# waiwera/waiwera

Hardware: AMD Instinct MI355X
Metric: Newton steps/sec, 10M-cell eos_we (BCSR SpMV GB/s in roofline) (higher is better)
Workload: dtype f64

## Files before the change

### include/waiwera_hip_bench.h

```cpp
#ifndef WAIWERA_HIP_BENCH_H
#define WAIWERA_HIP_BENCH_H
#include "waiwera_hip.h"
#ifdef __cplusplus
extern "C" {
#endif

int wai_comm_stats(wai_ctx *ctx, long long *allreduces, long long *exchanges);
int wai_gather_stats(wai_ctx *ctx, long long *gathers);
int wai_launch_stats(wai_ctx *ctx, long long *kernels, long long *copies);
int wai_tracer_stats(wai_ctx *ctx, long long *assembly_sweeps);

int wai_bench_mute_comm(wai_ctx *ctx, int on);
int wai_test_drop_partials(wai_ctx *ctx, int n);
int wai_test_drop_stream_wait(wai_ctx *ctx, int which);
int wai_test_device_memory(long long *allocations, long long *bytes);
int wai_test_pc_operator(wai_ctx *ctx, int spmv, const double *x, const double *x2, double alpha, int dot_mode,
                         const double *aux, int split, int fin_phase, const double *scal_in, double *z, double *scal_out);
int wai_pc_axpy_capable(wai_ctx *ctx);
int wai_test_partial_count(wai_ctx *ctx);
int wai_test_desc_templates(wai_ctx *ctx, int *bricks, int *rows);
enum { WAI_KV_DOT = 0, WAI_KV_DOTS, WAI_KV_WAXPY, WAI_KV_BCGS_P, WAI_KV_BCGS_S, WAI_KV_BCGS_XR, WAI_KV_BCGS_XRP,
       WAI_KV_BCGS_XRP_DERIVE, WAI_KV_SCALARS, WAI_KV_MDOT, WAI_KV_MAXPY_NORM, WAI_KV_SCALE_TO, WAI_KV_UPDATE_X };
int wai_test_krylov_vec(wai_ctx *ctx, int op, int variant, int n, int k, long long ld, long long len, double alpha,
                        double *vecs, double *basis, const double *coef, double *scal, double *post);
int wai_halo_size(wai_ctx *ctx, int dof, long long *bytes_sent, int *n_neighbours);

int wai_timer_start(wai_ctx *ctx);
int wai_timer_stop(wai_ctx *ctx, float *ms);
int wai_bench_kernel(wai_ctx *ctx, int which, int reps, float *ms_per_launch);
int wai_bcgs_composed(wai_ctx *ctx);
int wai_profile_enable(wai_ctx *ctx, int on);
int wai_profile_get(wai_ctx *ctx, int kclass, double *ms, long long *launches);
int wai_profile_reset(wai_ctx *ctx);

#ifdef __cplusplus
}
#endif
#endif
```

### waiwera_amd/csrc/context.hpp

```cpp
#pragma once
#include <hip/hip_runtime.h>
#include <string>
#include <type_traits>
#include <vector>
#include "../../include/waiwera_hip.h"
#include "devbuf.hpp"
#include "ilu_schedule.hpp"
#include "mesh_pattern.hpp"
#include "physics.hip.h"

namespace wai {

__host__ __device__ __forceinline__ size_t ell_ld(size_t n) {
  size_t ld = (n + 511) & ~(size_t)511;
  if ((ld & 262143) == 0) ld += 512;
  return ld;
}
__host__ __device__ __forceinline__ size_t ell_rows(int bs, size_t n) {
  if (bs >= 3) return ell_ld(n);
  return n;
}
__host__ __device__ __forceinline__ size_t ell_ix1(int bs, size_t n, int r, int k, size_t i) {
  if (bs >= 3) return ((i >> 6) * (size_t)(bs * bs) + (size_t)(r * bs + k)) * 64 + (i & 63);
  return ((size_t)r * n + i) * bs + k;
// ... 119 lines not shown
  std::vector<int> h_rowptr, h_colidx;
};

struct LinSys;
struct IluSchedule : ScheduleFacts {
  DevBuf<int> sub_ptr;
  DevBuf<int> sub_nlev;
  DevBuf<int> sub_split;
  DevBuf<int> row_info;
  DevBuf<unsigned long long> row_infow;
  DevBuf<double> fval;
  DevBuf<double> dinv;
  DevBuf<int> row_uoff;
  DevBuf<int> row_tslot;
  DevBuf<int> sub_int;
  DevBuf<int> sub_bnd;
  DevBuf<int> sub_order;
  DevBuf<int> row_uoffw;
  DevBuf<unsigned short> col16;
  DevBuf<int> sub_seg;
  DevBuf<int> t_info, t_uoff;
  DevBuf<unsigned short> t_col16;
  DevBuf<int> sub_desc;
  DevBuf<int> ord_f;
  DevBuf<int> ord_b;
  const LinSys* owner = nullptr;
};
inline int pc_threads(const IluSchedule& s) { return ((s.max_rows + 63) / 64) * 64; }

template <class F>
int with_bs(int bs, F&& f) {
  switch (bs) {
    case 1: f(std::integral_constant<int, 1>{}); return 0;
    case 2: f(std::integral_constant<int, 2>{}); return 0;
    case 3: f(std::integral_constant<int, 3>{}); return 0;
    case 4: f(std::integral_constant<int, 4>{}); return 0;
    default: return -1;
  }
}
template <class F>
void with_flag(bool flag, F&& f) {
  if (flag) f(std::true_type{});
  else f(std::false_type{});
}
template <class F>
int with_eos(int kind, F&& f) {
// ... 176 lines not shown
  wai::Network net;
  std::vector<int> src_gidx;
  int src_nglobal = 0;
  wai::Pattern pat;
  wai::LinSys flow, aux, coupled;
  wai::KrylovVecs kv, kv_coupled;
  wai::IluSchedule ilu;
  wai::LuBlocks lu;
  wai::Krylov ks;
  wai::Tracers tr;
  wai::Gather gat;
  wai::DevBuf<double> tr_bc, tr_inj, tr_rhsb;
  wai::DevBuf<double> flu, flu_last_iter, flu_last_step, flu_pert;
  wai::DevBuf<double> hstep;
  wai::DevBuf<double> w_y, w_yold, w_delta, w_f, w_lhs, w_a, w_b, w_c;
  wai::DevBuf<int> d_flags;
  wai::PinnedBuf<int> h_flags;
  wai::DevBuf<double> d_red;
  wai::PinnedBuf<double> h_red;
  wai::DevBuf<double> stage[4];
  size_t stage_len = 0;
  struct EnvSw {
    bool fin_separate = false; bool no_col16 = false; bool scalar_kernels = false; bool iluk_level_path = false;
    bool asm_unfused = false; bool no_desc_share = false;
  } env;
  int test_drop_wait = 0;
  int n_nbr = 0;
  std::vector<int> nbr_rank, send_ptr, recv_ptr;
  wai::DevBuf<int> d_send_idx; wai::DevBuf<double> d_sendbuf, d_recvbuf;
  int send_total = 0, max_dof_buf = 0;
  double fnorm0 = 0.0;
  int method = 0;
  double ratio = 0.0;
  wai::DevBuf<double> w_lhs2;
  int scheme = 0, taken = 0;
  double dt_last = 0.0;
  wai::DevBuf<double> w_hist;
  wai::DevBuf<double> w_hist_prev;
  double dt_last_prev = 0.0;
  bool can_reject = false;
  bool prof_on = false;
  bool last_iter_partial = false;
  double prof_ms[wai::KC_COUNT] = {0};
  long long prof_n[wai::KC_COUNT] = {0};
  std::string err;
  bool bc_set = false;
  int dbg = 0;
// ... 80 lines not shown
```

### waiwera_amd/csrc/ilu_schedule.hpp

```cpp
#pragma once
#include <algorithm>
#include <numeric>
#include <string>
#include <unordered_map>
#include <vector>

namespace wai {

struct ScheduleFacts {
  int nsub = 0, max_rows = 0, max_lev = 0;
  std::vector<int> sub;
  bool wide = false;
  bool diag_only = false;
  bool scaled = true;
  bool park = true;
  int max_nl = 0;
  int n_int = 0, n_bnd = 0;
  int max_ublocks = 0;
  int max_ublocks_w = 0;
  bool fast3 = false;
  int max_nlu = 0;
  bool rows_kernel = false;
  bool wave_kernel = false;
  int n_templates = 0, template_rows = 0;
  bool big = false;
  bool sublu = false;
  int nlev_f = 0, nlev_b = 0;
  std::vector<int> lev_f_ptr, lev_b_ptr;
};

struct HostSchedule : ScheduleFacts {
  std::vector<int> nlev;
  std::vector<int> info;
  std::vector<unsigned long long> infow;
  std::vector<int> uoff;
  std::vector<int> uoffw;
  std::vector<int> tslot;
  std::vector<int> split;
  std::vector<int> order;
  std::vector<int> sub_int, sub_bnd;
  std::vector<int> ord_f, ord_b;
  std::vector<unsigned short> c16;
  std::vector<int> seg;
  std::vector<int> t_info, t_uoff;
  std::vector<unsigned short> t_c16;
  std::vector<int> desc;
};

struct ScheduleOpts {
  bool ghosts = false;
  bool allow_wide = true, sublu = false, fill = false;
  int mesh_W = 0;
  bool box_faces = false;
  int max_seg = 8;
  bool ilu_general = false;
  int pc_rows = -1;
  bool pc_wave = true;
};

struct ScheduleCsr {
  const std::vector<int>& rowptr;
  const std::vector<int>& colidx;
  const int* row(int i) const { return colidx.data() + rowptr[i]; }
  int count(int i) const { return rowptr[i + 1] - rowptr[i]; }
};
struct ScheduleRows {
  std::vector<int> diag, lfirst, ulast, levf, levb;
  int max_nu = 0, nlf_all = 0, nlb_all = 0;
  bool offdiag_fill = false;
// ... 51 lines not shown
      const int k = row[q];
      const int* rk = A.row(k);
      const int* e = std::lower_bound(rk + r.diag[k] + 1, rk + r.ulast[k], i);
      const int r2 = (e < rk + r.ulast[k] && *e == i) ? (int)(e - rk) : 15;
      pack |= (r2 & 15) << (4 * p);
    }
    out.tslot[i] = pack;
    out.max_nl = std::max(out.max_nl, r.diag[i] - r.lfirst[i]);
  }
}

inline void sub_upper_offsets(int lo, int hi, ScheduleRows& r, HostSchedule& out) {
  int ucount = 0, ucountw = 0;
  for (int i = lo; i < hi; i++) {
    const int nL = r.diag[i] - r.lfirst[i], nU = r.ulast[i] - r.diag[i] - 1;
    if (nL > 3 || nU > 3 || r.lfirst[i] > 3 || r.diag[i] > 3) out.fast3 = false;
    out.max_nlu = std::max(out.max_nlu, std::max(nL, nU));
    out.uoff[i] = ucount;
    ucount += std::min(nU, 3);
    out.uoffw[i] = ucountw;
    ucountw += nU;
    r.max_nu = std::max(r.max_nu, nU);
  }
  out.max_ublocks = std::max(out.max_ublocks, ucount);
  out.max_ublocks_w = std::max(out.max_ublocks_w, ucountw);
}

inline void schedule_rows(const ScheduleCsr& A, int N, ScheduleRows& r, HostSchedule& out) {
  r.diag.resize(N); r.lfirst.resize(N); r.ulast.resize(N); r.levf.resize(N); r.levb.resize(N);
  for (int i = 0; i < N; i++) r.diag[i] = (int)(std::lower_bound(A.row(i), A.row(i) + A.count(i), i) - A.row(i));
  out.nlev.assign(out.nsub, 0);
  out.uoff.assign(N, 0); out.uoffw.assign(N, 0); out.tslot.assign(N, 0);
  out.fast3 = true;
  for (int sd = 0; sd < out.nsub; sd++) {
    const int lo = out.sub[sd], hi = out.sub[sd + 1];
    out.max_rows = std::max(out.max_rows, hi - lo);
    int nlf, nlb;
    sub_slots_and_levels(A, lo, hi, r, nlf, nlb);
    if (!r.offdiag_fill) r.offdiag_fill = sub_offdiag_fill(A, lo, hi, r);
    sub_tslot(A, lo, hi, r, out);
    sub_upper_offsets(lo, hi, r, out);
    out.nlev[sd] = (nlf & 0xffff) | (nlb << 16);
    out.max_lev = std::max(out.max_lev, std::max(nlf, nlb));
    r.nlf_all = std::max(r.nlf_all, nlf); r.nlb_all = std::max(r.nlb_all, nlb);
  }
}
// ... 142 lines not shown
}

inline void descriptor_templates(HostSchedule& out) {
  std::unordered_map<std::string, int> seen;
  auto bytes = [](const void* p, size_t n) { return std::string(static_cast<const char*>(p), n); };
  out.desc.resize(out.nsub);
  for (int sd = 0; sd < out.nsub; sd++) {
    const int lo = out.sub[sd], R = out.sub[sd + 1] - lo;
    const std::string key = bytes(&R, sizeof(int)) + bytes(out.info.data() + lo, sizeof(int) * R) +
                            bytes(out.uoff.data() + lo, sizeof(int) * R) +
                            bytes(out.c16.data() + (size_t)lo * 8, sizeof(unsigned short) * 8 * R);
    const auto it = seen.emplace(key, (int)out.t_info.size());
    if (it.second) {
      out.n_templates++;
      out.t_info.insert(out.t_info.end(), out.info.begin() + lo, out.info.begin() + lo + R);
      out.t_uoff.insert(out.t_uoff.end(), out.uoff.begin() + lo, out.uoff.begin() + lo + R);
      out.t_c16.insert(out.t_c16.end(), out.c16.begin() + (size_t)lo * 8, out.c16.begin() + (size_t)(lo + R) * 8);
    }
    out.desc[sd] = it.first->second;
  }
  out.template_rows = (int)out.t_info.size();
}

inline int build_host_schedule(const std::vector<int>& rowptr, const std::vector<int>& colidx, const std::vector<int>& sub,
                               int N, int W, int np, const ScheduleOpts& opts, HostSchedule& out, std::string& err) {
  out = HostSchedule();
  if (sub.empty() || sub.front() != 0 || sub.back() != N) { err = "sub_ptr must cover [0, n_owned]"; return -2; }
  if (!std::is_sorted(sub.begin(), sub.end())) { err = "sub_ptr not monotone"; return -2; }
  out.sub = sub;
  out.nsub = (int)sub.size() - 1;
  const ScheduleCsr A{rowptr, colidx};
  ScheduleRows r;
  schedule_rows(A, N, r, out);
  if (int e = schedule_descriptors(N, W, np, opts, r, out, err)) return e;
  launch_order(out);
  if (opts.ghosts) interior_and_face_lists(A, N, opts.box_faces, out);
  if ((out.big || out.wide) && !opts.sublu) level_sets(N, r, out);
  select_kernels(W, np, opts, r, out);
  if (out.rows_kernel) rows_split_record(A, W, out);
  if (park_serves(out, np) && col16_indices(A, N, W, opts.max_seg, out)) descriptor_templates(out);
  return 0;
}

}
```

### waiwera_amd/csrc/kernels_fused.hip

```cpp
#include "pc_generic.hip.h"
#include "pc_wide.hip.h"
#include "pc_park.hip.h"
#include "pc_rows.hip.h"
#include "pc_wave.hip.h"
#include "krylov_vec.hip.h"

namespace wai {

static inline int vgrid(int n) {
  int g = (n + TPB - 1) / TPB;
  return g > 1024 ? 1024 : (g < 1 ? 1 : g);
}

void read_env(wai_ctx* c) {
  c->env.fin_separate = getenv("WAI_FIN_SEPARATE") != nullptr;
  c->env.no_col16 = getenv("WAI_NO_COL16") != nullptr;
  c->env.scalar_kernels = getenv("WAI_BCGS_SCALAR_KERNELS") != nullptr;
  c->env.iluk_level_path = getenv("WAI_ILUK_LEVEL_PATH") != nullptr;
  c->env.asm_unfused = getenv("WAI_ASM_UNFUSED") != nullptr;
  c->env.no_desc_share = getenv("WAI_NO_DESC_SHARE") != nullptr;
}

int pc_kernel_kind(const wai_ctx* c, const Bcsr& J, const IluSchedule& s) {
  if (J.dg) return -1;
  if (s.wide) return 4;
  if (c->dbg) return 0;
  if (s.wave_kernel && J.bs >= 3) return 3;
  if (s.rows_kernel) return 2;
  if (park_serves(s, J.bs)) return 1;
  return 0;
}
static bool kind_composes(int kind) { return kind >= 1 && kind <= 3; }
bool pc_axpy_capable(const wai_ctx* c, const Bcsr& M) { return !c->ilu.big && kind_composes(pc_kernel_kind(c, M, c->ilu)); }
bool pc_axpy_default(const wai_ctx* c, const Bcsr& M) {
  if (c->ilu.big) return false;
  const int kind = pc_kernel_kind(c, M, c->ilu);
  return (kind == 1 && c->ilu.col16 && !c->env.no_col16) || kind == 3;
}

template <int BS>
static void launch_pc_bs(wai_ctx* c, const Bcsr& J, const IluSchedule& s, bool spmv, const double* in, double* z,
                         int dot_mode, const double* aux, const int* list, int nrun, const Fin* finp, const double* in2,
                         const Bcsr* F, const int* row_map) {
  if (!list) { nrun = s.nsub; list = s.sub_order; }
  const bool with_fin = finp && dot_mode != 0;
  Fin fin;
  if (finp && dot_mode != 0) { fin = *finp; fin.count = nrun; fin.nb = s.nsub; fin.nf = fin_slices(s.nsub); }
  c->ks.n_launch++;
  const int grid = ((nrun + 7) / 8) * 8 + (with_fin ? fin.nf : 0), T = pc_threads(s);
  const size_t lds = ((size_t)T * BS + 80) * sizeof(double);
  auto sp_ax = [&](auto&& go) {
    if (spmv) with_flag(in2 != nullptr, [&](auto ax) { go(std::true_type{}, ax); });
    else go(std::false_type{}, std::false_type{});
  };
  const int kind = pc_kernel_kind(c, J, s);
  const double* scal = c->ks.scal;
  const int* rp = (size_t)J.nnzb * 10 < (size_t)J.n * J.W * 9 ? J.rowptr : nullptr;
  if (kind == 4) {
    constexpr int NSB = BS == 1 ? 8 : (BS == 2 ? 6 : 0);
    if constexpr (BS == 2) {
      if (F && row_map && s.max_nlu <= 3) {
        with_flag(spmv, [&](auto sp) {
          hipLaunchKernelGGL((k_pc_wide<2, decltype(sp)::value, true, 3, true>), grid, T, lds, c->stream, J.n, J.W, nrun, s.sub_ptr,
                             s.sub_nlev, s.row_infow, s.row_uoffw, J.col, rp, J.val, s.fval, in, z, aux, c->ks.partials, c->ks.nb_max,
                             dot_mode, 0, list, fin, F->col, F->n, row_map);
        });
// ... 55 lines not shown
        constexpr int NLU = decltype(nlu)::value;
        hipLaunchKernelGGL((k_pc_rows<BS, decltype(sp)::value, NLU, NLU, decltype(ax)::value>), grid, TR, lds_r, c->stream, J.n, J.W,
                           nrun, s.sub_ptr, s.sub_nlev, s.row_info, J.col, s.fval, s.dinv, in, in2, scal, z, aux, c->ks.partials,
                           c->ks.nb_max, dot_mode, list, rp, s.sub_split, fin);
      });
    };
    if (s.max_nlu <= 3) rows(std::integral_constant<int, 3>{});
    else rows(std::integral_constant<int, 4>{});
    return;
  }
  if constexpr (BS == 2) {
    if (kind == 1) {
      const size_t lds_park = lds + (size_t)s.max_ublocks * 4 * sizeof(double);
      Stagger stagger;
      stagger.ncu = c->n_cu;
      stagger.per_cu = std::max(1, std::min(3, (int)((size_t)160 * 1024 / (lds_park + 704))));
      stagger.ticks = 600;
      const bool on16 = s.col16 && !c->env.no_col16;
      const bool shared = on16 && s.sub_desc && !c->env.no_desc_share;
      const int* d_info = shared ? s.t_info.get() : s.row_info.get();
      const int* d_uoff = shared ? s.t_uoff.get() : s.row_uoff.get();
      const unsigned short* d_c16 = shared ? s.t_col16.get() : s.col16.get();
      const int* d_desc = shared ? s.sub_desc.get() : s.sub_ptr.get();
      with_flag(on16, [&](auto c16) {
        sp_ax([&](auto sp, auto ax) {
          hipLaunchKernelGGL((k_pc_park<decltype(sp)::value, decltype(ax)::value, decltype(c16)::value>), grid, T, lds_park, c->stream,
                             J.n, J.W, nrun, s.sub_ptr, s.sub_nlev, d_desc, d_info, d_uoff, J.col, d_c16, s.sub_seg, s.fval, s.dinv,
                             in, in2, scal, z, aux, c->ks.partials, c->ks.nb_max, dot_mode, list, fin, stagger);
        });
      });
      return;
    }
  }
  auto generic = [&](auto di) {
    with_flag(spmv, [&](auto sp) {
      with_flag(s.fast3, [&](auto fast) {
        hipLaunchKernelGGL((k_pc<BS, decltype(sp)::value, decltype(di)::value, decltype(fast)::value>), grid, T, lds, c->stream,
                           J.n, J.W, nrun, s.sub_ptr, s.sub_nlev, s.row_info, J.col, J.val, s.fval, s.dinv, in, z, aux,
                           c->ks.partials, c->ks.nb_max, dot_mode, c->dbg, list, fin);
      });
    });
  };
  if (s.diag_only && s.scaled) generic(std::integral_constant<int, 2>{});
  else if (s.diag_only) generic(std::integral_constant<int, 1>{});
  else generic(std::integral_constant<int, 0>{});
}
// ... 205 lines not shown
```

### waiwera_amd/csrc/measure.hip

```cpp
#include "host.hpp"

using namespace wai;

namespace {
typedef double stream_d2 __attribute__((ext_vector_type(2)));
__global__ __launch_bounds__(256) void k_stream_copy(const stream_d2* __restrict__ src, stream_d2* __restrict__ dst, size_t n2) {
  const size_t stride = (size_t)gridDim.x * 256;
  size_t i = (size_t)blockIdx.x * 256 + threadIdx.x;
  for (; i + stride < n2; i += 2 * stride) {
    const stream_d2 a = __builtin_nontemporal_load(src + i), b = __builtin_nontemporal_load(src + i + stride);
    __builtin_nontemporal_store(a, dst + i);
    __builtin_nontemporal_store(b, dst + i + stride);
  }
  if (i < n2) __builtin_nontemporal_store(__builtin_nontemporal_load(src + i), dst + i);
}
__global__ __launch_bounds__(256) void k_stream_read(const stream_d2* __restrict__ src, size_t n2, double* sink) {
  const size_t stride = (size_t)gridDim.x * 256;
  size_t i = (size_t)blockIdx.x * 256 + threadIdx.x;
  double t = 0.0;
  for (; i + stride < n2; i += 2 * stride) {
    const stream_d2 a = __builtin_nontemporal_load(src + i), b = __builtin_nontemporal_load(src + i + stride);
    t += (a.x + a.y) + (b.x + b.y);
  }
  if (i < n2) { const stream_d2 a = __builtin_nontemporal_load(src + i); t += a.x + a.y; }
// ... 215 lines not shown
    e = launch_pc_split(c, sys.A, k.R, k.T, dot_mode, a, fp, v, nullptr);
  } else if (spmv) {
    e = pc_amul(c, sys, k.R, k.T, dot_mode, a, fin_phase, v, false);
  } else {
    e = pc_solve(c, sys, k.R, k.T, dot_mode, k.R, a, fin_phase);
  }
  if (e) return e;
  if (fin_phase == -2 && dot_mode)
    vec_finalize(c, c->ks.nb_pc, pc_dot_slot0(dot_mode), pc_dot_nslots(dot_mode), -1);
  HIPCHK(c, hipMemcpyAsync(z, k.T, n * sizeof(double), hipMemcpyDefault, c->stream));
  HIPCHK(c, hipMemcpyAsync(s, c->ks.scal, sizeof(s), hipMemcpyDeviceToHost, c->stream));
  HIPCHK(c, hipStreamSynchronize(c->stream));
  for (int i = 0; i < 16; i++) scal_out[i] = s[i];
  return 0;
}
int wai_pc_axpy_capable(wai_ctx* c) { return c ? (pc_operand_composable(c) ? 1 : 0) : -2; }
int wai_test_partial_count(wai_ctx* c) { return c ? c->ks.nb_pc : -2; }
int wai_test_desc_templates(wai_ctx* c, int* bricks, int* rows) {
  if (!c) return -2;
  const bool have = c->ilu.sub_desc != nullptr;
  if (bricks) *bricks = c->ilu.nsub;
  if (rows) *rows = have ? c->ilu.template_rows : 0;
  return have ? c->ilu.n_templates : 0;
}
int wai_test_krylov_vec(wai_ctx* c, int op, int variant, int n, int k, long long ld, long long len, double alpha, double* vecs,
                        double* basis, const double* coef, double* scal, double* post) {
  if (!c || !vecs || !scal || !post) return -2;
  const bool gmres = op == WAI_KV_MDOT || op == WAI_KV_MAXPY_NORM || op == WAI_KV_UPDATE_X;
  auto refuse = [&](const char* why) { c->err = std::string("wai_test_krylov_vec: ") + why; return -2; };
  if (op < WAI_KV_DOT || op > WAI_KV_UPDATE_X) return refuse("no such op");
  if (n < 1) return refuse("n < 1");
  if (k < 0 || k > MAX_RESTART || (gmres && k < 1)) return refuse("basis count out of range");
  if (len < (long long)n) return refuse("len < n");
  if (gmres && (ld < (long long)n || !basis)) return refuse("ld < n, or no basis");
  if (op == WAI_KV_UPDATE_X && !coef) return refuse("no coefficients");
  const int vmax[] = {0, 1, 2, 0, 0, 3, 0, 0, 6, 0, 0, 1, 0};
  if (variant < 0 || variant > vmax[op] || (op == WAI_KV_SCALARS && variant == 1)) return refuse("no such variant");
  read_env(c);
  enum { X, R, RP, P, V, S, T, NV };
  KrylovVecs kv;
  DevBuf<double>* own[NV] = {&kv.X_own, &kv.R, &kv.RP, &kv.P, &kv.V, &kv.S, &kv.T};
  const size_t L = (size_t)len, nbasis = gmres ? (size_t)(k + 1) * (size_t)ld : 0;
  for (int i = 0; i < NV; i++) {
    if (own[i]->alloc(c, L)) return -1;
    HIPCHK(c, hipMemcpyAsync(own[i]->get(), vecs + (size_t)i * L, L * sizeof(double), hipMemcpyHostToDevice, c->stream));
  }
// ... 90 lines not shown
```

### waiwera_amd/csrc/pc_park.hip.h

```cpp
#pragma once
#include "reductions.hip.h"

namespace wai {

template <bool SPMV, bool AX, bool C16>
__global__ __launch_bounds__(512, 6) void k_pc_park(
    int n, int W, int nsub, const int* __restrict__ sub_ptr, const int* __restrict__ sub_nlev,
    const int* __restrict__ sub_desc, const int* __restrict__ row_info, const int* __restrict__ row_uoff, const int* __restrict__ col,
    const unsigned short* __restrict__ col16, const int* __restrict__ sub_seg,
    const double* __restrict__ sval, const double* __restrict__ dinv, const double* __restrict__ in,
    const double* __restrict__ in2, const double* __restrict__ scal,
    double* __restrict__ z, const double* __restrict__ aux, double* partials, int nb_max, int dot,
    const int* __restrict__ sub_list, Fin fin, Stagger stagger) {
  constexpr int BS = 2, BB = 4, MLU = 3;
  extern __shared__ __attribute__((aligned(16))) double lds[];
  if (fin_block(fin, partials, nb_max)) return;
  int s = xcd_remap(blockIdx.x, nsub);
  if (s >= nsub) return;
  if (sub_list) s = sub_list[s];
  const int lo = sub_ptr[s], R = sub_ptr[s + 1] - lo;
  int dlo = lo;
  if constexpr (C16) dlo = sub_desc[s];
  const int nl = sub_nlev[s];
  const int nlf = nl & 0xffff, nlb = nl >> 16;
  const int tid = threadIdx.x, i = lo + tid, di = dlo + tid;
  const bool active = tid < R;
  const double nalpha = AX ? -scal[S_ALPHA] : 0.0;
  stagger_start(stagger);
  double* ys = lds;
  double* upark = lds + (size_t)blockDim.x * BS + 80;
  double Lf[MLU][BB];
  int Lc[MLU], Uc[MLU], lf = -1, lb = -1, uo = 0, nU = 0;
  double xin[BS] = {0.0, 0.0}, avp[BS] = {0.0, 0.0};
#pragma unroll
  for (int p = 0; p < MLU; p++) {
    Lc[p] = tid; Uc[p] = tid;
#pragma unroll
    for (int e = 0; e < BB; e++) Lf[p][e] = 0.0;
  }
  int lfirst = 0, dslot = 0, ulast = 0;
  int cgs[WMAX];
  if (active) {
    unpack_info(row_info[di], lfirst, dslot, ulast, lf, lb);
    uo = row_uoff[di];
    nU = ulast - dslot - 1;
    if constexpr (C16) {
      const int* sg = sub_seg + (size_t)s * 8;
      const int g0 = sg[0], g1 = sg[1], g2 = sg[2], g3 = sg[3], g4 = sg[4], g5 = sg[5], g6 = sg[6], g7 = sg[7];
      typedef unsigned wai_u4v __attribute__((ext_vector_type(4)));
      const wai_u4v pk = reinterpret_cast<const wai_u4v*>(col16)[di];
      const unsigned pw[4] = {pk.x, pk.y, pk.z, pk.w};
      unsigned cu[WMAX];
#pragma unroll
// ... 14 lines not shown
      }
    }
  }
  double acc[BS] = {0.0, 0.0};
  if (active) {
#pragma unroll
    for (int q = 0; q < WMAX; q++) {
      if (q < W) {
        const int cg = cgs[q];
        double blk[BB];
        load_block<BS>(sval, n, q, i, blk);
        if constexpr (SPMV) {
          double xv[BS];
          load_xs<BS, AX>(in, in2, nalpha, cg, xv);
          acc[0] += blk[0] * xv[0] + blk[1] * xv[1];
          acc[1] += blk[2] * xv[0] + blk[3] * xv[1];
          xin[0] = q == dslot ? xv[0] : xin[0];
          xin[1] = q == dslot ? xv[1] : xin[1];
        }
        const bool isl = (q >= lfirst) && (q < dslot), isu = (q > dslot) && (q < ulast);
#pragma unroll
        for (int p = 0; p < MLU; p++) {
          const bool tl = isl && (q - lfirst == p), tu = isu && (q - dslot - 1 == p);
          Lc[p] = tl ? cg - lo : Lc[p];
          Uc[p] = tu ? cg - lo : Uc[p];
#pragma unroll
          for (int e = 0; e < BB; e++) Lf[p][e] = tl ? blk[e] : Lf[p][e];
        }
        if (isu) {
          double* dst = upark + (size_t)(uo + (q - dslot - 1)) * BB;
          *reinterpret_cast<double2*>(dst) = make_double2(blk[0], blk[1]);
          *reinterpret_cast<double2*>(dst + 2) = make_double2(blk[2], blk[3]);
        }
      }
    }
    if constexpr (!SPMV) {
      double r[BS], dv[BB];
      load_x<BS>(in, i, r);
      load_pivot<BS>(dinv, n, i, dv);
      acc[0] = dv[0] * r[0] + dv[1] * r[1];
      acc[1] = dv[2] * r[0] + dv[3] * r[1];
      xin[0] = r[0]; xin[1] = r[1];
    }
    if (dot == PC_DOT_ZA || dot == PC_DOT_MERGED) load_x_stream<BS>(aux, i, avp);
  }
  if (active) *reinterpret_cast<double2*>(ys + tid * 2) = make_double2(acc[0], acc[1]);
  __syncthreads();
  auto gather3 = [&](const int (&cc)[MLU], const double (&ff)[MLU][BB], double* sum) {
// ... 24 lines not shown
    const double2 u0 = *reinterpret_cast<const double2*>(src), u1 = *reinterpret_cast<const double2*>(src + 2);
    Lf[p][0] = have ? u0.x : 0.0; Lf[p][1] = have ? u0.y : 0.0;
    Lf[p][2] = have ? u1.x : 0.0; Lf[p][3] = have ? u1.y : 0.0;
  }
  double out[BS] = {0.0, 0.0};
  for (int lev = 0; lev < nlb; lev++) {
    if (lb == lev) {
      const double2 a = *reinterpret_cast<const double2*>(ys + tid * 2);
      double sum[BS];
      gather3(Uc, Lf, sum);
      out[0] = a.x - sum[0];
      out[1] = a.y - sum[1];
      *reinterpret_cast<double2*>(ys + tid * 2) = make_double2(out[0], out[1]);
    }
    if (lev + 1 < nlb) __syncthreads();
  }
  if (active) store_z2(z, (size_t)i, out[0], out[1]);
  if (dot != 0) {
    double* red = lds + (size_t)blockDim.x * BS;
    double v[5] = {0.0, 0.0, 0.0, 0.0, 0.0};
    pc_row_dots<BS, true, false>(dot, v, out, active, [&](double (&x)[BS]) { x[0] = xin[0]; x[1] = xin[1]; },
                                 [&](double (&a)[BS]) { a[0] = avp[0]; a[1] = avp[1]; });
    __syncthreads();
    pc_reduce_dots(dot, v, red, partials, nb_max, s);
  }
}

}
```

### waiwera_amd/csrc/pc_setup.hip

```cpp
#include "host.hpp"
#include "asm_pattern.hpp"

using namespace wai;

namespace wai {

int build_schedule(wai_ctx* c, IluSchedule& s, const std::vector<int>& rowptr, const std::vector<int>& colidx,
                   const std::vector<int>& sub, int N, int W, int np, bool ghosts, bool allow_wide, bool sublu, bool fill) {
  ScheduleOpts o;
  o.ghosts = ghosts; o.allow_wide = allow_wide; o.sublu = sublu; o.fill = fill;
  o.mesh_W = c->pat.W;
  o.box_faces = c->mesh.n_halo == 0 && W == 7;
  if (const char* e = getenv("WAI_COL16_MAX_SEG")) o.max_seg = std::max(1, std::min(8, atoi(e)));
#ifdef WAI_ILU_GENERAL
  o.ilu_general = true;
#endif
#ifdef WAI_PC_ROWS
  o.pc_rows = WAI_PC_ROWS != 0;
#endif
#ifdef WAI_PC_WAVE
  o.pc_wave = WAI_PC_WAVE != 0;
#endif
  HostSchedule h;
  if (int e = build_host_schedule(rowptr, colidx, sub, N, W, np, o, h, c->err)) return e;
  static_cast<ScheduleFacts&>(s) = ScheduleFacts();
  auto put = [c](auto& buf, const auto& v) { buf.reset(); return !v.empty() && buf.upload(c, v); };
  if (put(s.sub_ptr, h.sub) || put(s.sub_nlev, h.nlev) || put(s.row_info, h.info) || put(s.row_infow, h.infow) ||
      put(s.row_uoff, h.uoff) || put(s.row_uoffw, h.uoffw) || put(s.row_tslot, h.tslot) || put(s.sub_split, h.split) ||
      put(s.sub_order, h.order) || put(s.sub_int, h.sub_int) || put(s.sub_bnd, h.sub_bnd) || put(s.ord_f, h.ord_f) ||
      put(s.ord_b, h.ord_b) || put(s.col16, h.c16) || put(s.sub_seg, h.seg) || put(s.t_info, h.t_info) ||
      put(s.t_uoff, h.t_uoff) || put(s.t_col16, h.t_c16) || put(s.sub_desc, h.desc))
    return -1;
  static_cast<ScheduleFacts&>(s) = std::move(h);
  if (s.fval.alloc(c, ell_size(np, N, W)) || s.dinv.alloc(c, (size_t)np * np * ell_rows(np, N))) return -1;
  return 0;
}

int ensure_halo_dof(wai_ctx* c, int dof) {
  if (dof <= c->max_dof_buf) return 0;
  c->max_dof_buf = dof;
  return c->d_sendbuf.alloc(c, (size_t)c->send_total * dof) || c->d_recvbuf.alloc(c, (size_t)c->mesh.n_halo * dof) ? -1 : 0;
}

int ghost_rows(wai_ctx* c, const LinSys& sys, std::vector<int>& grp, std::vector<int>& gci, std::vector<int>& gslot) {
  const Pattern& J = c->pat;
  const int N = J.n, H = c->mesh.n_halo, W = J.W;
  std::vector<double> ids((size_t)N + H, -1.0);
  const double base = (double)c->comm->rank * 4294967296.0;
  for (int i = 0; i < N; i++) ids[i] = base + i;
  double* scratch = sys.kv->tmp;
  HIPCHK(c, hipMemcpyAsync(scratch, ids.data(), sizeof(double) * (N + H), hipMemcpyHostToDevice, c->stream));
  if (halo_exchange(c, scratch, 1)) return -1;
  HIPCHK(c, hipMemcpyAsync(ids.data(), scratch, sizeof(double) * (N + H), hipMemcpyDeviceToHost, c->stream));
  HIPCHK(c, hipStreamSynchronize(c->stream));
// ... 182 lines not shown
```

### waiwera_amd/csrc/reductions.hip.h

```cpp
#pragma once
#include "linalg_device.hip.h"

namespace wai {

typedef unsigned wai_u4 __attribute__((ext_vector_type(4)));
__device__ __forceinline__ void post_scalars(const double* scal, double* post, int seq) {
  const double v0 = scal[S_DP2], v1 = 8.0 * (double)seq + scal[S_BREAK];
  const unsigned long long chk = (unsigned long long)__double_as_longlong(v0) ^ (unsigned long long)__double_as_longlong(v1) ^ POST_KEY;
#if defined(__gfx942__) || defined(__gfx950__)
  wai_u4 w;
  w.x = (unsigned)__double2loint(v0); w.y = (unsigned)__double2hiint(v0);
  w.z = (unsigned)__double2loint(v1); w.w = (unsigned)__double2hiint(v1);
  asm volatile("global_store_dwordx4 %0, %1, off sc0 sc1" : : "v"(post), "v"(w) : "memory");
#else
  __hip_atomic_store(reinterpret_cast<unsigned long long*>(post), (unsigned long long)__double_as_longlong(v0), __ATOMIC_RELAXED, __HIP_MEMORY_SCOPE_SYSTEM);
  __hip_atomic_store(reinterpret_cast<unsigned long long*>(post) + 1, (unsigned long long)__double_as_longlong(v1), __ATOMIC_RELAXED, __HIP_MEMORY_SCOPE_SYSTEM);
#endif
  __hip_atomic_store(reinterpret_cast<unsigned long long*>(post) + 2, chk, __ATOMIC_RELAXED, __HIP_MEMORY_SCOPE_SYSTEM);
}
__device__ __forceinline__ void derive_merged(double* s) {
  const double st = s[S_D1], tt = s[S_D2], ss = s[S_DP2], srp = s[S_RHONEW], trp = s[S_W2];
  if (tt == 0.0) { s[S_BREAK] = 2.0; s[S_OMEGA] = 0.0; }
  else s[S_OMEGA] = st / tt;
  const double om = s[S_OMEGA];
// ... 212 lines not shown
    if (lane == 0 && w < NS) {
      double t = 0.0;
      for (int q = 0; q < nw; q++) t += red[w * 16 + q];
      store_partial(partials + (size_t)(slot0 + w) * nb_max + blk, t);
    }
    return;
  }
  if (threadIdx.x == 0) {
#pragma unroll
    for (int s = 0; s < NS; s++) {
      double t = 0.0;
      for (int q = 0; q < nw; q++) t += red[s * 16 + q];
      store_partial(partials + (size_t)(slot0 + s) * nb_max + blk, t);
    }
  }
}
__device__ __forceinline__ void pc_reduce_dots(int mode, double (&v)[5], double* red, double* partials, int nb_max, int blk) {
  const int slot0 = pc_dot_slot0(mode);
  if (mode == PC_DOT_MERGED) wg_reduce_store<5>(v, red, partials, nb_max, slot0, blk);
  else if (mode == PC_DOT_XZ) { double v2[2] = {v[0], v[1]}; wg_reduce_store<2>(v2, red, partials, nb_max, slot0, blk); }
  else { double v1[1] = {v[0]}; wg_reduce_store<1>(v1, red, partials, nb_max, slot0, blk); }
}

template <int N, bool SUM, bool GUARD2, class GetX, class GetA>
__device__ __forceinline__ void pc_row_dots(int mode, double (&v)[5], const double (&o)[N], bool active, GetX get_x,
                                            GetA get_a) {
  auto dot = [&](int q, const double (&p)[N], const double (&r)[N]) {
    if constexpr (SUM) {
      double t = p[0] * r[0];
#pragma unroll
      for (int k = 1; k < N; k++) t += p[k] * r[k];
      v[q] = t;
    } else {
#pragma unroll
      for (int k = 0; k < N; k++) v[q] += p[k] * r[k];
    }
  };
  double x[N], a[N];
  if (mode == PC_DOT_ZA) {
    if (active) { get_a(a); dot(0, o, a); }
  } else if (mode == PC_DOT_XZ) {
    if (active || !GUARD2) { get_x(x); dot(0, x, o); dot(1, o, o); }
  } else if (mode == PC_DOT_MERGED) {
    if (active) { get_x(x); get_a(a); dot(0, x, o); dot(1, o, o); dot(2, x, x); dot(3, x, a); dot(4, o, a); }
  } else {
    dot(0, o, o);
// ... 26 lines not shown
```

### waiwera_amd/flow_simulation.py

```python
import ctypes as C

import numpy as np

from . import lib as _lib
from .lib import LIB, WaiError


class FlowSimulation:
    def __init__(self, mesh, eos="we", opts=None, device=0, temperature=20.0,
                 relperm=("linear", [0.0, 1.0, 0.0, 1.0]), capillary=("zero", []), thermo="iapws",
                 permeability_modifier=None):
        self.mesh = mesh
        self.eos_name = eos
        self._keep = dict(
            face_cells=_lib._i32(mesh.face_cells), face_geom=_lib._f64(mesh.face_geom),
            cell_geom=_lib._f64(mesh.cell_geom), rock=_lib._f64(mesh.rock),
            sub_ptr=_lib._i32(mesh.sub_ptr) if mesh.sub_ptr is not None else None)
        k = self._keep
        md = _lib.MeshDesc()
        md.n_owned, md.n_halo, md.n_bc, md.n_faces = mesh.n_owned, mesh.n_halo, mesh.n_bc, mesh.n_faces
        md.face_cells = k["face_cells"].ctypes.data_as(_lib.pi)
        md.face_geom = k["face_geom"].ctypes.data_as(_lib.pd)
        md.cell_geom = k["cell_geom"].ctypes.data_as(_lib.pd)
        md.rock = k["rock"].ctypes.data_as(_lib.pd)
# ... 329 lines not shown
    def pc_operator(self, x, x2=None, alpha=0.0, dot_mode=0, aux=None, spmv=True, split=False, fin_phase=-2, scal_in=None):
        xi = _lib._f64(x)
        x2i = _lib._f64(x2) if x2 is not None else None
        ai = _lib._f64(aux) if aux is not None else None
        s_in = _lib._f64(np.zeros(16) if scal_in is None else scal_in)
        assert xi.size == self.num_dof and s_in.size == 16
        z, s_out = np.zeros(self.num_dof), np.zeros(16)
        self._chk(LIB.wai_test_pc_operator(self.h, 1 if spmv else 0, _lib.ptr(xi), _lib.ptr(x2i), float(alpha), int(dot_mode),
                                           _lib.ptr(ai), 1 if split else 0, int(fin_phase), s_in.ctypes.data_as(_lib.pd),
                                           _lib.ptr(z), s_out.ctypes.data_as(_lib.pd)), "test_pc_operator")
        return z, s_out

    def pc_axpy_capable(self):
        return LIB.wai_pc_axpy_capable(self.h) == 1

    def partial_count(self):
        return self._chk(LIB.wai_test_partial_count(self.h), "test_partial_count")

    def desc_templates(self):
        nb, nr = C.c_int(0), C.c_int(0)
        nt = self._chk(LIB.wai_test_desc_templates(self.h, C.byref(nb), C.byref(nr)), "test_desc_templates")
        return nt, nb.value, nr.value

    KV_OPS = ("dot", "dots", "waxpy", "bcgs_p", "bcgs_s", "bcgs_xr", "bcgs_xrp", "bcgs_xrp_derive", "scalars", "mdot",
              "maxpy_norm", "scale_to", "update_x")
    KV_VECS = ("X", "R", "RP", "P", "V", "S", "T")

    def krylov_vec(self, op, n, vecs, scal, variant=0, k=0, ld=0, basis=None, coef=None, alpha=0.0):
        v = np.array(vecs, dtype=np.float64, order="C")
        s = np.array(scal, dtype=np.float64)
        assert v.ndim == 2 and v.shape[0] == len(self.KV_VECS) and s.shape == (128,)
        b = np.array(basis, dtype=np.float64).ravel() if basis is not None else None
        assert b is None or b.size == (k + 1) * ld
        cf = _lib._f64(coef) if coef is not None else None
        assert cf is None or cf.size >= k
        post = np.full(2, np.nan)
        P = lambda a: a.ctypes.data_as(_lib.pd) if a is not None else None
        self._chk(LIB.wai_test_krylov_vec(self.h, self.KV_OPS.index(op), int(variant), int(n), int(k), int(ld), v.shape[1],
                                          float(alpha), P(v), P(b), P(cf), P(s), P(post)), "test_krylov_vec")
        return v, b, s, post

    def ksp_solve(self, b, x):
        its, reason, rn = C.c_int(0), C.c_int(0), C.c_double(0)
        self._chk(LIB.wai_ksp_solve(self.h, _lib.ptr(b), _lib.ptr(x), C.byref(its), C.byref(reason),
                                    C.byref(rn)), "ksp_solve")
        return its.value, reason.value, rn.value
# ... 121 lines not shown
```

### waiwera_amd/lib.py

```python
import ctypes as C
import os

import numpy as np

HERE = os.path.dirname(os.path.abspath(__file__))
LIB_PATH = os.path.join(HERE, "libwaiwera_hip.so")

EOS_W, EOS_WE, EOS_WCE, EOS_WSE, EOS_WAE, EOS_WSCE, EOS_WSAE = 0, 1, 2, 3, 4, 5, 6
EOS_KIND = {"w": EOS_W, "we": EOS_WE, "wce": EOS_WCE, "wse": EOS_WSE, "wae": EOS_WAE, "wsce": EOS_WSCE,
            "wsae": EOS_WSAE}
RP = {"fully_mobile": 0, "fully mobile": 0, "linear": 1, "pickens": 2, "corey": 3, "grant": 4,
      "van_genuchten": 5, "van genuchten": 5, "table": 6}
CP = {"zero": 0, "linear": 1, "van_genuchten": 2, "van genuchten": 2, "table": 3}
INTERP = {"linear": 0, "step": 1, "pchip": 2}
KSP = {"bcgs": 0, "gmres": 1, "bcgsl": 2, "lgmres": 3}
PC = {"bjacobi": 0, "asm": 1, "none": 2, "lu": 3}
KCLASS = ["eos", "residual", "jacobian", "spmv", "pc_apply", "pc_setup", "vector", "transitions"]

d, i32 = C.c_double, C.c_int
pd, pi = C.POINTER(C.c_double), C.POINTER(C.c_int)


THERMO = {"iapws": 0, "ifc67": 1}
TRACER_SOLVE = {"per_tracer": 0, "coupled": 1}
# ... 104 lines not shown
        "wai_num_fluid_dof": (i32, [vp]),
        "wai_get_fluxes": (i32, [vp, vp]),
        "wai_num_flux_dof": (i32, [vp]),
        "wai_get_source_separated": (i32, [vp, pd]),
        "wai_block_size": (i32, [vp]),
        "wai_set_halo": (i32, [vp, i32, pi, pi, pi, pi]),
        "wai_comm_unique_id": (i32, [C.c_char_p]),
        "wai_comm_init": (i32, [vp, i32, i32, C.c_char_p]),
        "wai_halo_exchange": (i32, [vp, vp, i32]),
        "wai_comm_size": (i32, [vp]),
        "wai_comm_stats": (i32, [vp, C.POINTER(C.c_longlong), C.POINTER(C.c_longlong)]),
        "wai_gather_stats": (i32, [vp, C.POINTER(C.c_longlong)]),
        "wai_gather_rows": (i32, [vp, i32, i32, vp, i32, vp, i32, vp]),
        "wai_gather_fluid": (i32, [vp, i32, i32, i32, pi, vp, i32, vp]),
        "wai_launch_stats": (i32, [vp, C.POINTER(C.c_longlong), C.POINTER(C.c_longlong)]),
        "wai_bench_mute_comm": (i32, [vp, i32]),
        "wai_test_drop_partials": (i32, [vp, i32]),
        "wai_test_drop_stream_wait": (i32, [vp, i32]),
        "wai_test_device_memory": (i32, [C.POINTER(C.c_longlong), C.POINTER(C.c_longlong)]),
        "wai_test_pc_operator": (i32, [vp, i32, vp, vp, d, i32, vp, i32, i32, pd, vp, pd]),
        "wai_pc_axpy_capable": (i32, [vp]),
        "wai_test_partial_count": (i32, [vp]),
        "wai_test_desc_templates": (i32, [vp, C.POINTER(i32), C.POINTER(i32)]),
        "wai_test_krylov_vec": (i32, [vp, i32, i32, i32, i32, C.c_longlong, C.c_longlong, d, pd, pd, pd, pd, pd]),
        "wai_halo_size": (i32, [vp, i32, C.POINTER(C.c_longlong), C.POINTER(i32)]),
        "wai_pc_kernel_name": (C.c_char_p, [vp]),
        "wai_pre_timestep": (i32, [vp]),
        "wai_pre_retry_timestep": (i32, [vp]),
        "wai_pre_iteration": (i32, [vp]),
        "wai_pre_eval": (i32, [vp, d, vp]),
        "wai_lhs": (i32, [vp, d, vp, vp]),
        "wai_rhs": (i32, [vp, d, vp, vp]),
        "wai_post_linesearch": (i32, [vp, vp, vp, vp, pi, pi]),
        "wai_set_residual_form": (i32, [vp, i32, d, vp]),
        "wai_set_timestep_method": (i32, [vp, i32]),
        "wai_residual": (i32, [vp, d, d, vp, vp, vp]),
        "wai_jacobian": (i32, [vp, d, d, vp, vp]),
        "wai_jacobian_nnzb": (i32, [vp]),
        "wai_jacobian_pattern": (i32, [vp, pi, pi]),
        "wai_jacobian_get_values": (i32, [vp, vp]),
        "wai_jacobian_set_values": (i32, [vp, vp]),
        "wai_spmv": (i32, [vp, vp, vp]),
        "wai_pc_setup": (i32, [vp]),
        "wai_pc_apply": (i32, [vp, vp, vp]),
        "wai_ksp_solve": (i32, [vp, vp, vp, pi, pi, pd]),
        "wai_max_scaled": (i32, [vp, vp, vp, d, pd, pi]),
# ... 160 lines not shown
```

Before: 5.173.

## Pack short ILU subdomains into shared workgroups in park preconditioner kernel

Adds host-side bin packing of subdomains whose thread count is below the maximum block size, so several short subdomains share one workgroup, each wave reading a per-wave record of subdomain, thread offset, upper-block base and group level counts. The park PC kernel gains a PACK variant that uses these records, offsets LDS upper-block storage, and reduces dot products per wave range. The goal is to cut idle threads and workgroup count when subdomain sizes vary. In exchange, all members of a group run to the group's maximum level count and there is extra per-wave indexing, plus a test hook and an env opt-out.

```diff
diff --git a/include/waiwera_hip_bench.h b/include/waiwera_hip_bench.h
--- a/include/waiwera_hip_bench.h
+++ b/include/waiwera_hip_bench.h
@@ -19,6 +19,7 @@
 int wai_pc_axpy_capable(wai_ctx *ctx);
 int wai_test_partial_count(wai_ctx *ctx);
 int wai_test_desc_templates(wai_ctx *ctx, int *bricks, int *rows);
+int wai_test_pack_groups(wai_ctx *ctx, int list, int *shared, int *table, int cap);
 enum { WAI_KV_DOT = 0, WAI_KV_DOTS, WAI_KV_WAXPY, WAI_KV_BCGS_P, WAI_KV_BCGS_S, WAI_KV_BCGS_XR, WAI_KV_BCGS_XRP,
        WAI_KV_BCGS_XRP_DERIVE, WAI_KV_SCALARS, WAI_KV_MDOT, WAI_KV_MAXPY_NORM, WAI_KV_SCALE_TO, WAI_KV_UPDATE_X };
 int wai_test_krylov_vec(wai_ctx *ctx, int op, int variant, int n, int k, long long ld, long long len, double alpha,
diff --git a/waiwera_amd/csrc/context.hpp b/waiwera_amd/csrc/context.hpp
--- a/waiwera_amd/csrc/context.hpp
+++ b/waiwera_amd/csrc/context.hpp
@@ -165,6 +165,7 @@
   DevBuf<int> t_info, t_uoff;
   DevBuf<unsigned short> t_col16;
   DevBuf<int> sub_desc;
+  DevBuf<int> pack_tab[3];
   DevBuf<int> ord_f;
   DevBuf<int> ord_b;
   const LinSys* owner = nullptr;
@@ -387,7 +388,7 @@
   size_t stage_len = 0;
   struct EnvSw {
     bool fin_separate = false; bool no_col16 = false; bool scalar_kernels = false; bool iluk_level_path = false;
-    bool asm_unfused = false; bool no_desc_share = false;
+    bool asm_unfused = false; bool no_desc_share = false; bool no_pack = false;
   } env;
   int test_drop_wait = 0;
   int n_nbr = 0;
diff --git a/waiwera_amd/csrc/ilu_schedule.hpp b/waiwera_amd/csrc/ilu_schedule.hpp
--- a/waiwera_amd/csrc/ilu_schedule.hpp
+++ b/waiwera_amd/csrc/ilu_schedule.hpp
@@ -23,6 +23,7 @@
   bool rows_kernel = false;
   bool wave_kernel = false;
   int n_templates = 0, template_rows = 0;
+  int n_groups[3] = {0, 0, 0}, n_shared[3] = {0, 0, 0};
   bool big = false;
   bool sublu = false;
   int nlev_f = 0, nlev_b = 0;
@@ -45,6 +46,8 @@
   std::vector<int> t_info, t_uoff;
   std::vector<unsigned short> t_c16;
   std::vector<int> desc;
+  std::vector<int> ucount;
+  std::vector<int> groups[3];
 };
 
 struct ScheduleOpts {
@@ -142,6 +145,7 @@
     ucountw += nU;
     r.max_nu = std::max(r.max_nu, nU);
   }
+  out.ucount.push_back(ucount);
   out.max_ublocks = std::max(out.max_ublocks, ucount);
   out.max_ublocks_w = std::max(out.max_ublocks_w, ucountw);
 }
@@ -330,6 +334,74 @@
   out.template_rows = (int)out.t_info.size();
 }
 
+constexpr int PACK_WAVES = 8, PACK_REC = 4;
+inline void pack_list(const HostSchedule& s, std::vector<int> list, std::vector<int>& table, int& n_groups, int& n_shared) {
+  table.clear(); n_groups = 0; n_shared = 0;
+  const int T = ((s.max_rows + 63) / 64) * 64;
+  auto rows = [&](int sd) { return s.sub[sd + 1] - s.sub[sd]; };
+  auto threads = [&](int sd) { return ((rows(sd) + 63) / 64) * 64; };
+  if (T > 64 * PACK_WAVES) return;
+  std::sort(list.begin(), list.end());
+  std::vector<int> shorts;
+  for (int sd : list) if (threads(sd) < T) shorts.push_back(sd);
+  std::stable_sort(shorts.begin(), shorts.end(), [&](int a, int b) { return rows(a) > rows(b); });
+  struct Bin { std::vector<int> members; int threads = 0, ublocks = 0; };
+  std::vector<Bin> bins;
+  std::unordered_map<int, int> opens;
+  bool any = false;
+  for (int sd : shorts) {
+    size_t b = 0;
+    while (b < bins.size() && (bins[b].threads + threads(sd) > T || bins[b].ublocks + s.ucount[sd] > s.max_ublocks)) b++;
+    if (b == bins.size()) { bins.emplace_back(); opens[sd] = (int)b; }
+    else any = true;
+    bins[b].members.push_back(sd); bins[b].threads += threads(sd); bins[b].ublocks += s.ucount[sd];
+  }
+  if (!any) return;
+  std::vector<std::vector<int>> groups;
+  for (int sd : list) {
+    if (threads(sd) >= T) groups.push_back({sd});
+    else if (opens.count(sd)) groups.push_back(bins[opens[sd]].members);
+  }
+  auto levels = [&](const std::vector<int>& g, int& nlf, int& nlb) {
+    nlf = 0; nlb = 0;
+    for (int sd : g) { nlf = std::max(nlf, s.nlev[sd] & 0xffff); nlb = std::max(nlb, s.nlev[sd] >> 16); }
+  };
+  auto cost = [&](const std::vector<int>& g) {
+    int nlf, nlb, r = 0;
+    levels(g, nlf, nlb);
+    for (int sd : g) r += rows(sd);
+    return (nlf + nlb) * 4096 + r;
+  };
+  const int n = (int)groups.size(), per = (n + 7) >> 3;
+  for (int j = 0; j < 8; j++) {
+    const int a = std::min(j * per, n), b = std::min((j + 1) * per, n);
+    std::stable_sort(groups.begin() + a, groups.begin() + b,
+                     [&](const std::vector<int>& x, const std::vector<int>& y) { return cost(x) > cost(y); });
+  }
+  table.assign((size_t)n * PACK_WAVES * PACK_REC, 0);
+  for (int g = 0; g < n; g++) {
+    int nlf, nlb, toff = 0, ubase = 0;
+    levels(groups[g], nlf, nlb);
+    int* rec = table.data() + (size_t)g * PACK_WAVES * PACK_REC;
+    for (int w = 0; w < PACK_WAVES; w++) { rec[w * PACK_REC] = -1; rec[w * PACK_REC + 1] = w * 64; rec[w * PACK_REC + 3] = nlf | (nlb << 16); }
+    for (int sd : groups[g]) {
+      for (int w = toff / 64; w < (toff + threads(sd)) / 64; w++) {
+        rec[w * PACK_REC] = sd; rec[w * PACK_REC + 1] = toff; rec[w * PACK_REC + 2] = ubase;
+      }
+      toff += threads(sd); ubase += s.ucount[sd];
+    }
+    if (groups[g].size() > 1) n_shared += (int)groups[g].size();
+  }
+  n_groups = n;
+}
+inline void pack_groups(HostSchedule& out) {
+  std::vector<int> all(out.nsub);
+  std::iota(all.begin(), all.end(), 0);
+  pack_list(out, all, out.groups[0], out.n_groups[0], out.n_shared[0]);
+  if (!out.sub_int.empty()) pack_list(out, out.sub_int, out.groups[1], out.n_groups[1], out.n_shared[1]);
+  if (!out.sub_bnd.empty()) pack_list(out, out.sub_bnd, out.groups[2], out.n_groups[2], out.n_shared[2]);
+}
+
 inline int build_host_schedule(const std::vector<int>& rowptr, const std::vector<int>& colidx, const std::vector<int>& sub,
                                int N, int W, int np, const ScheduleOpts& opts, HostSchedule& out, std::string& err) {
   out = HostSchedule();
@@ -347,6 +419,7 @@
   select_kernels(W, np, opts, r, out);
   if (out.rows_kernel) rows_split_record(A, W, out);
   if (park_serves(out, np) && col16_indices(A, N, W, opts.max_seg, out)) descriptor_templates(out);
+  if (park_serves(out, np)) pack_groups(out);
   return 0;
 }
 
diff --git a/waiwera_amd/csrc/kernels_fused.hip b/waiwera_amd/csrc/kernels_fused.hip
--- a/waiwera_amd/csrc/kernels_fused.hip
+++ b/waiwera_amd/csrc/kernels_fused.hip
@@ -19,6 +19,7 @@
   c->env.iluk_level_path = getenv("WAI_ILUK_LEVEL_PATH") != nullptr;
   c->env.asm_unfused = getenv("WAI_ASM_UNFUSED") != nullptr;
   c->env.no_desc_share = getenv("WAI_NO_DESC_SHARE") != nullptr;
+  c->env.no_pack = getenv("WAI_NO_PACK") != nullptr;
 }
 
 int pc_kernel_kind(const wai_ctx* c, const Bcsr& J, const IluSchedule& s) {
@@ -42,6 +43,7 @@
 static void launch_pc_bs(wai_ctx* c, const Bcsr& J, const IluSchedule& s, bool spmv, const double* in, double* z,
                          int dot_mode, const double* aux, const int* list, int nrun, const Fin* finp, const double* in2,
                          const Bcsr* F, const int* row_map) {
+  const int which = !list ? 0 : (list == s.sub_int ? 1 : (list == s.sub_bnd ? 2 : -1));
   if (!list) { nrun = s.nsub; list = s.sub_order; }
   const bool with_fin = finp && dot_mode != 0;
   Fin fin;
@@ -143,6 +145,15 @@
       const int* d_uoff = shared ? s.t_uoff.get() : s.row_uoff.get();
       const unsigned short* d_c16 = shared ? s.t_col16.get() : s.col16.get();
       const int* d_desc = shared ? s.sub_desc.get() : s.sub_ptr.get();
+      if (shared && which >= 0 && s.pack_tab[which] && !c->env.no_pack) {
+        const int ngrp = s.n_groups[which], gridp = ((ngrp + 7) / 8) * 8 + (with_fin ? fin.nf : 0);
+        sp_ax([&](auto sp, auto ax) {
+          hipLaunchKernelGGL((k_pc_park<decltype(sp)::value, decltype(ax)::value, true, true>), gridp, T, lds_park, c->stream,
+                             J.n, J.W, ngrp, s.sub_ptr, s.sub_nlev, d_desc, d_info, d_uoff, J.col, d_c16, s.sub_seg, s.fval, s.dinv,
+                             in, in2, scal, z, aux, c->ks.partials, c->ks.nb_max, dot_mode, s.pack_tab[which].get(), fin, stagger);
+        });
+        return;
+      }
       with_flag(on16, [&](auto c16) {
         sp_ax([&](auto sp, auto ax) {
           hipLaunchKernelGGL((k_pc_park<decltype(sp)::value, decltype(ax)::value, decltype(c16)::value>), grid, T, lds_park, c->stream,
diff --git a/waiwera_amd/csrc/measure.hip b/waiwera_amd/csrc/measure.hip
--- a/waiwera_amd/csrc/measure.hip
+++ b/waiwera_amd/csrc/measure.hip
@@ -261,6 +261,18 @@
   if (bricks) *bricks = c->ilu.nsub;
   if (rows) *rows = have ? c->ilu.template_rows : 0;
   return have ? c->ilu.n_templates : 0;
+}
+int wai_test_pack_groups(wai_ctx* c, int list, int* shared, int* table, int cap) {
+  if (!c || list < 0 || list > 2 || cap < 0 || (cap > 0 && !table)) return -2;
+  read_env(c);
+  const IluSchedule& s = c->ilu;
+  const bool packed = !s.big && pc_kernel_kind(c, c->flow.A, s) == 1 && s.col16 && !c->env.no_col16 && s.sub_desc &&
+                      !c->env.no_desc_share && s.pack_tab[list] && !c->env.no_pack;
+  if (shared) *shared = packed ? s.n_shared[list] : 0;
+  if (!packed) return 0;
+  const int n = std::min(cap, s.n_groups[list] * 32);
+  if (n > 0) HIPCHK(c, hipMemcpy(table, s.pack_tab[list].get(), sizeof(int) * n, hipMemcpyDeviceToHost));
+  return s.n_groups[list];
 }
 int wai_test_krylov_vec(wai_ctx* c, int op, int variant, int n, int k, long long ld, long long len, double alpha, double* vecs,
                         double* basis, const double* coef, double* scal, double* post) {
diff --git a/waiwera_amd/csrc/pc_park.hip.h b/waiwera_amd/csrc/pc_park.hip.h
--- a/waiwera_amd/csrc/pc_park.hip.h
+++ b/waiwera_amd/csrc/pc_park.hip.h
@@ -3,7 +3,7 @@
 
 namespace wai {
 
-template <bool SPMV, bool AX, bool C16>
+template <bool SPMV, bool AX, bool C16, bool PACK = false>
 __global__ __launch_bounds__(512, 6) void k_pc_park(
     int n, int W, int nsub, const int* __restrict__ sub_ptr, const int* __restrict__ sub_nlev,
     const int* __restrict__ sub_desc, const int* __restrict__ row_info, const int* __restrict__ row_uoff, const int* __restrict__ col,
@@ -17,18 +17,26 @@
   if (fin_block(fin, partials, nb_max)) return;
   int s = xcd_remap(blockIdx.x, nsub);
   if (s >= nsub) return;
-  if (sub_list) s = sub_list[s];
-  const int lo = sub_ptr[s], R = sub_ptr[s + 1] - lo;
+  int toff = 0, ubase = 0, nl_grp = 0;
+  if constexpr (PACK) {
+    const int w = __builtin_amdgcn_readfirstlane((int)threadIdx.x >> 6);
+    const int4 rec = reinterpret_cast<const int4*>(sub_list)[(size_t)s * 8 + w];
+    s = rec.x; toff = rec.y; ubase = rec.z; nl_grp = rec.w;
+  } else {
+    if (sub_list) s = sub_list[s];
+  }
+  const bool member = !PACK || s >= 0;
+  const int lo = member ? sub_ptr[s] : 0, R = member ? sub_ptr[s + 1] - lo : 0;
   int dlo = lo;
-  if constexpr (C16) dlo = sub_desc[s];
-  const int nl = sub_nlev[s];
+  if constexpr (C16) dlo = member ? sub_desc[s] : 0;
+  const int nl = PACK ? nl_grp : sub_nlev[s];
   const int nlf = nl & 0xffff, nlb = nl >> 16;
-  const int tid = threadIdx.x, i = lo + tid, di = dlo + tid;
-  const bool active = tid < R;
+  const int tid = threadIdx.x, lob = lo - toff, i = lob + tid, di = dlo - toff + tid;
+  const bool active = tid - toff < R;
   const double nalpha = AX ? -scal[S_ALPHA] : 0.0;
   stagger_start(stagger);
   double* ys = lds;
-  double* upark = lds + (size_t)blockDim.x * BS + 80;
+  double* upark = lds + (size_t)blockDim.x * BS + 80 + (size_t)ubase * BB;
   double Lf[MLU][BB];
   int Lc[MLU], Uc[MLU], lf = -1, lb = -1, uo = 0, nU = 0;
   double xin[BS] = {0.0, 0.0}, avp[BS] = {0.0, 0.0};
@@ -89,8 +97,8 @@
 #pragma unroll
         for (int p = 0; p < MLU; p++) {
           const bool tl = isl && (q - lfirst == p), tu = isu && (q - dslot - 1 == p);
-          Lc[p] = tl ? cg - lo : Lc[p];
-          Uc[p] = tu ? cg - lo : Uc[p];
+          Lc[p] = tl ? cg - lob : Lc[p];
+          Uc[p] = tu ? cg - lob : Uc[p];
 #pragma unroll
           for (int e = 0; e < BB; e++) Lf[p][e] = tl ? blk[e] : Lf[p][e];
         }
@@ -161,7 +169,8 @@
     pc_row_dots<BS, true, false>(dot, v, out, active, [&](double (&x)[BS]) { x[0] = xin[0]; x[1] = xin[1]; },
                                  [&](double (&a)[BS]) { a[0] = avp[0]; a[1] = avp[1]; });
     __syncthreads();
-    pc_reduce_dots(dot, v, red, partials, nb_max, s);
+    if constexpr (PACK) pc_reduce_dots_waves(dot, v, red, partials, nb_max, s, toff >> 6, (R + 63) >> 6);
+    else pc_reduce_dots(dot, v, red, partials, nb_max, s);
   }
 }
 
diff --git a/waiwera_amd/csrc/pc_setup.hip b/waiwera_amd/csrc/pc_setup.hip
--- a/waiwera_amd/csrc/pc_setup.hip
+++ b/waiwera_amd/csrc/pc_setup.hip
@@ -29,7 +29,8 @@
       put(s.row_uoff, h.uoff) || put(s.row_uoffw, h.uoffw) || put(s.row_tslot, h.tslot) || put(s.sub_split, h.split) ||
       put(s.sub_order, h.order) || put(s.sub_int, h.sub_int) || put(s.sub_bnd, h.sub_bnd) || put(s.ord_f, h.ord_f) ||
       put(s.ord_b, h.ord_b) || put(s.col16, h.c16) || put(s.sub_seg, h.seg) || put(s.t_info, h.t_info) ||
-      put(s.t_uoff, h.t_uoff) || put(s.t_col16, h.t_c16) || put(s.sub_desc, h.desc))
+      put(s.t_uoff, h.t_uoff) || put(s.t_col16, h.t_c16) || put(s.sub_desc, h.desc) || put(s.pack_tab[0], h.groups[0]) ||
+      put(s.pack_tab[1], h.groups[1]) || put(s.pack_tab[2], h.groups[2]))
     return -1;
   static_cast<ScheduleFacts&>(s) = std::move(h);
   if (s.fval.alloc(c, ell_size(np, N, W)) || s.dinv.alloc(c, (size_t)np * np * ell_rows(np, N))) return -1;
diff --git a/waiwera_amd/csrc/reductions.hip.h b/waiwera_amd/csrc/reductions.hip.h
--- a/waiwera_amd/csrc/reductions.hip.h
+++ b/waiwera_amd/csrc/reductions.hip.h
@@ -258,6 +258,43 @@
   else { double v1[1] = {v[0]}; wg_reduce_store<1>(v1, red, partials, nb_max, slot0, blk); }
 }
 
+template <int NS>
+__device__ __forceinline__ void wg_reduce_store_waves(double (&v)[NS], double* red, double* partials, int nb_max, int slot0,
+                                                      int blk, int w0, int nwm) {
+  const int lane = threadIdx.x & 63, w = threadIdx.x >> 6;
+#pragma unroll
+  for (int s = 0; s < NS; s++) {
+    const double t = wave_sum(v[s]);
+    if (lane == 0) red[s * 16 + w] = t;
+  }
+  __syncthreads();
+  if (blk < 0 || lane != 0) return;
+  const int k = w - w0;
+  if (nwm >= NS) {
+    if (k < NS) {
+      double t = 0.0;
+      for (int q = w0; q < w0 + nwm; q++) t += red[k * 16 + q];
+      store_partial(partials + (size_t)(slot0 + k) * nb_max + blk, t);
+    }
+    return;
+  }
+  if (k == 0) {
+#pragma unroll
+    for (int s = 0; s < NS; s++) {
+      double t = 0.0;
+      for (int q = w0; q < w0 + nwm; q++) t += red[s * 16 + q];
+      store_partial(partials + (size_t)(slot0 + s) * nb_max + blk, t);
+    }
+  }
+}
+__device__ __forceinline__ void pc_reduce_dots_waves(int mode, double (&v)[5], double* red, double* partials, int nb_max, int blk,
+                                                     int w0, int nwm) {
+  const int slot0 = pc_dot_slot0(mode);
+  if (mode == PC_DOT_MERGED) wg_reduce_store_waves<5>(v, red, partials, nb_max, slot0, blk, w0, nwm);
+  else if (mode == PC_DOT_XZ) { double v2[2] = {v[0], v[1]}; wg_reduce_store_waves<2>(v2, red, partials, nb_max, slot0, blk, w0, nwm); }
+  else { double v1[1] = {v[0]}; wg_reduce_store_waves<1>(v1, red, partials, nb_max, slot0, blk, w0, nwm); }
+}
+
 template <int N, bool SUM, bool GUARD2, class GetX, class GetA>
 __device__ __forceinline__ void pc_row_dots(int mode, double (&v)[5], const double (&o)[N], bool active, GetX get_x,
                                             GetA get_a) {
diff --git a/waiwera_amd/flow_simulation.py b/waiwera_amd/flow_simulation.py
--- a/waiwera_amd/flow_simulation.py
+++ b/waiwera_amd/flow_simulation.py
@@ -375,6 +375,15 @@
         nt = self._chk(LIB.wai_test_desc_templates(self.h, C.byref(nb), C.byref(nr)), "test_desc_templates")
         return nt, nb.value, nr.value
 
+    def pack_groups(self, which=0):
+        shared = C.c_int(0)
+        ng = self._chk(LIB.wai_test_pack_groups(self.h, which, C.byref(shared), None, 0), "test_pack_groups")
+        table = np.zeros(ng * 32, dtype=np.int32)
+        if ng:
+            self._chk(LIB.wai_test_pack_groups(self.h, which, C.byref(shared), table.ctypes.data_as(C.POINTER(C.c_int)), table.size),
+                      "test_pack_groups")
+        return ng, shared.value, table.reshape(ng, 8, 4)
+
     KV_OPS = ("dot", "dots", "waxpy", "bcgs_p", "bcgs_s", "bcgs_xr", "bcgs_xrp", "bcgs_xrp_derive", "scalars", "mdot",
               "maxpy_norm", "scale_to", "update_x")
     KV_VECS = ("X", "R", "RP", "P", "V", "S", "T")
diff --git a/waiwera_amd/lib.py b/waiwera_amd/lib.py
--- a/waiwera_amd/lib.py
+++ b/waiwera_amd/lib.py
@@ -150,6 +150,7 @@
         "wai_pc_axpy_capable": (i32, [vp]),
         "wai_test_partial_count": (i32, [vp]),
         "wai_test_desc_templates": (i32, [vp, C.POINTER(i32), C.POINTER(i32)]),
+        "wai_test_pack_groups": (i32, [vp, i32, C.POINTER(i32), C.POINTER(i32), i32]),
         "wai_test_krylov_vec": (i32, [vp, i32, i32, i32, i32, C.c_longlong, C.c_longlong, d, pd, pd, pd, pd, pd]),
         "wai_halo_size": (i32, [vp, i32, C.POINTER(C.c_longlong), C.POINTER(i32)]),
         "wai_pc_kernel_name": (C.c_char_p, [vp]),
```

After: 5.352, median of 6. +3.5%, better.
